# hyye/lio-mapping

Measured on AMD Instinct MI355X. Metric: sliding-window solves/sec, 64-line 130k-pt scans, window=15 (opt_window=5), higher is better.
Workload: dtype f64 (solve) / f32 (features); 1 GPU; HDL-64E outdoor_test_config_64, S_outdoor ray-cast scans, window_size=15 opt_window_size=5, one SolveOptimization per step, clouds resident in HBM; n_lidar_residuals=78236, local_map_points=76752, surf_stack_points=19386, parallelism=1 window

## Files before the change

### lio-mapping_amd/csrc/cloud_kernels.h

```cpp
#pragma once
#include <algorithm>
#include <cmath>
#include <cstdint>

#include "dev.h"
#include "hmath.h"

namespace lio {

struct VoxParams {
  float mn[3], mx[3];
  int minb[3], divb[3];
  int overflow;
  int n_valid;
};

struct Affine3f { float m[12]; };

#define LIO_MAX_FRAMES 32

struct ConcatSeg { const float4 *src; int n; int dst_off; int identity; int set_intensity; float intensity; Affine3f tf; };
struct ConcatArgs { ConcatSeg seg[LIO_MAX_FRAMES]; int nseg; int total; };
void launch_transform_concat(const ConcatArgs &a, float4 *dst, hipStream_t s);

void launch_deskew_to_end(float4 *pts, int n, const float q[4], const float p[3], float time_factor, hipStream_t s, bool keep_intensity = false);
void launch_rigid_map(const float4 *in, int n, const float q[4], const float p[3], float4 *out, hipStream_t s);

inline int cloud_bounds_blocks(int n) { return std::max(1, std::min(cdiv(n, 256), 512)); }
struct BoundsSeg { const float4 *pts; int n, nb, off; };
void launch_seg_bounds(const BoundsSeg *d_segs, int nseg, int max_nb, float *partial, float inv_leaf, VoxParams *d_out, hipStream_t s);

#define VSORT_CAP 4096
#define VSORT_MEAN 384
#define VSORT_OVERSAMPLE 8
#define VSORT_MAX_BUCKETS 1024
#define VSORT_MAX_N (VSORT_MAX_BUCKETS * VSORT_MEAN)
enum VoxSortPath { VSORT_PATH_SAMPLE = 0, VSORT_PATH_SINGLE = 1, VSORT_PATH_LIBRARY = 2 };
inline int vsort_buckets(size_t n) { return int((n + VSORT_MEAN - 1) / VSORT_MEAN); }

class VoxelGridDev {
 public:
  void sort_stats(unsigned long long out[3]) const { for (int k = 0; k < 3; ++k) out[k] = n_path_[k]; }
  int sort_pairs_hook(const uint32_t *keys, size_t n, uint32_t *keys_out, uint32_t *vals_out, hipStream_t s);
  size_t run(const float4 *in, size_t n, float leaf, DBuf<float4> &out, hipStream_t s, VoxParams *host_params = nullptr);
  void launch(const float4 *in, size_t n, float leaf, DBuf<float4> &out, hipStream_t s);
  size_t finish(VoxParams *host_params = nullptr);
  void set_host_signal(bool on) { use_signal_ = on; }
  VoxelGridDev() = default;
  VoxelGridDev(const VoxelGridDev &) = delete;
  VoxelGridDev &operator=(const VoxelGridDev &) = delete;

 private:
  const float4 *p_in_ = nullptr; size_t p_n_ = 0; DBuf<float4> *p_out_ = nullptr; hipStream_t p_stream_ = nullptr;
  float p_leaf_ = 0.f;
  void enqueue(bool exact, bool library);
  void reserve_sort(size_t n, hipStream_t s);
  int enqueue_sort(size_t n, hipStream_t s, bool library);
  DBuf<uint32_t> splitters_;
  DBuf<int> fill_;
  DBuf<unsigned long long> pairs_;
  int last_path_ = VSORT_PATH_LIBRARY;
  unsigned long long n_path_[3] = {0, 0, 0};
  HostBuf<char> h_mail_;
  int *h_count_ = nullptr;
  VoxParams *h_params_ = nullptr;
  DBuf<float> partial_;
  DBuf<VoxParams> params_;
  DBuf<uint32_t> keys_, keys2_, vals_, vals2_;
  DBuf<int> count_, tile_heads_;
  DBuf<char> tmp_;
  unsigned *h_flag_ = nullptr;
  unsigned seq_ = 0;
  HostSignal sig_{};
  bool use_signal_ = true;
};

struct GridDesc {
  int origin[3];
  int dims[3];
  float inv_cell;
  int n_points;
};

inline float knn_cell_edge(float min_match_sq_dis) { return std::sqrt(min_match_sq_dis) * 1.0001f + 1e-6f; }
inline float scan_to_map_cell_edge(float min_match_sq_dis) { return std::sqrt(min_match_sq_dis) * 1.0001f; }
inline void host_cloud_bounds(const float *xyzi, size_t n, float mn[3], float mx[3]) {
  for (int d = 0; d < 3; ++d) { mn[d] = 0.f; mx[d] = 0.f; }
  bool first = true;
  for (size_t i = 0; i < n; ++i) {
    const float *p = xyzi + 4 * i;
    if (!std::isfinite(p[0]) || !std::isfinite(p[1]) || !std::isfinite(p[2])) continue;
    for (int d = 0; d < 3; ++d) {
      if (first || p[d] < mn[d]) mn[d] = p[d];
      if (first || p[d] > mx[d]) mx[d] = p[d];
    }
    first = false;
  }
}
inline size_t grid_extent(GridDesc &g, const float mn[3], const float mx[3], float cell) {
  g.inv_cell = 1.0f / cell;
  size_t ncells = 1;
  for (int d = 0; d < 3; ++d) {
    const int lo = int(std::floor(mn[d] * g.inv_cell)) - 1, hi = int(std::floor(mx[d] * g.inv_cell)) + 1;
    g.origin[d] = lo; g.dims[d] = hi - lo + 1;
    ncells *= size_t(g.dims[d]);
  }
  return ncells;
}

class KnnGrid {
 public:
  void build(const float4 *pts, size_t n, const float mn[3], const float mx[3], float cell, hipStream_t s);
  const float4 *sorted() const { return sorted_.p; }
  const int *cells() const { return cells_.p; }
  const GridDesc &desc() const { return desc_; }

 private:
  GridDesc desc_{};
  DBuf<uint32_t> keys_, keys2_, vals_, vals2_;
  DBuf<float4> sorted_;
  DBuf<int> cells_, cnt_;
  bool cnt_dirty_ = false;
  DBuf<char> tmp_;
};

struct GridSeg { const float4 *pts; GridDesc g; int pt_off, cell_off, ncells; };
class GridBatch {
 public:
  void *begin(size_t head_bytes, int clouds);
  const void *head_dev() const { return d_tab_.p; }
  void add(const float4 *pts, int n);
  const VoxParams *bounds(hipStream_t s, float inv_leaf = 1.0f);
  void layout(float cell, size_t cells_cap);
  bool shared(int i) const { return gseg(i).pt_off >= 0; }
  const GridDesc &desc(int i) const { return gseg(i).g; }
  const float4 *sorted(int) const { return sorted_.p; }
  const int *cells(int i) const { return cells_.p + gseg(i).cell_off; }
// ... 149 lines not shown
```

### lio-mapping_amd/csrc/cloud_kernels.hip

```cpp
#include <cstring>
#include <hip/hip_runtime.h>
#include <rocprim/rocprim.hpp>

#include <cfloat>
#include <climits>

#include "cloud_kernels.h"
#include "cloud_device.h"

namespace lio {

__global__ void k_transform_concat(ConcatArgs a, float4 *__restrict__ dst) {
  int gid = blockIdx.x * blockDim.x + threadIdx.x;
  if (gid >= a.total) return;
  dst[gid] = concat_point(a.seg, a.nseg, gid, nullptr);
}

void launch_transform_concat(const ConcatArgs &a, float4 *dst, hipStream_t s) {
  if (a.total <= 0) return;
  hipLaunchKernelGGL(k_transform_concat, dim3(cdiv(a.total, 256)), dim3(256), 0, s, a, dst);
  LIO_HIP(hipGetLastError());
}

template <bool KEEP>
__global__ void __launch_bounds__(256) k_deskew_to_end(float4 *pts, int n, Quat<float> qe, Vec3<float> te, float time_factor) {
  int i = blockIdx.x * blockDim.x + threadIdx.x;
  if (i >= n) return;
  pts[i] = deskew_to_end_point<KEEP>(pts[i], qe, te, time_factor);
}
void launch_deskew_to_end(float4 *pts, int n, const float q[4], const float p[3], float time_factor, hipStream_t s, bool keep_intensity) {
  if (n <= 0) return;
  const Quat<float> qe(q[3], q[0], q[1], q[2]);
  const Vec3<float> te(p[0], p[1], p[2]);
  if (keep_intensity) hipLaunchKernelGGL(k_deskew_to_end<true>, dim3(cdiv(n, 256)), dim3(256), 0, s, pts, n, qe, te, time_factor);
  else hipLaunchKernelGGL(k_deskew_to_end<false>, dim3(cdiv(n, 256)), dim3(256), 0, s, pts, n, qe, te, time_factor);
  LIO_HIP(hipGetLastError());
}

__global__ void __launch_bounds__(256) k_rigid_map(const float4 *__restrict__ in, int n, Quat<float> q, Vec3<float> t, float4 *__restrict__ out) {
  const int i = blockIdx.x * blockDim.x + threadIdx.x;
  if (i >= n) return;
  out[i] = rigid_map_point(in[i], q, t);
}
void launch_rigid_map(const float4 *in, int n, const float q[4], const float p[3], float4 *out, hipStream_t s) {
  if (n <= 0) return;
  hipLaunchKernelGGL(k_rigid_map, dim3(cdiv(n, 256)), dim3(256), 0, s, in, n, Quat<float>(q[3], q[0], q[1], q[2]), Vec3<float>(p[0], p[1], p[2]), out);
  LIO_HIP(hipGetLastError());
}

__global__ void __launch_bounds__(VOX_TILE) k_seg_bounds(const BoundsSeg *__restrict__ recs, float *__restrict__ partial) {
  const BoundsSeg r = recs[blockIdx.y];
  if (int(blockIdx.x) >= r.nb) return;
  cloud_bounds_block(r.pts, r.n, blockIdx.x, r.nb, partial + (size_t(r.off) + blockIdx.x) * 8);
}
__global__ void __launch_bounds__(VOX_TILE) k_seg_bounds_fold(const BoundsSeg *__restrict__ recs, const float *__restrict__ partial, float inv_leaf,
                                                              VoxParams *__restrict__ out) {
  const BoundsSeg r = recs[blockIdx.x];
  VoxParams v;
  if (vox_fold_bounds(partial + size_t(r.off) * 8, r.nb, inv_leaf, v)) out[blockIdx.x] = v;
}
void launch_seg_bounds(const BoundsSeg *d_segs, int nseg, int max_nb, float *partial, float inv_leaf, VoxParams *d_out, hipStream_t s) {
  hipLaunchKernelGGL(k_seg_bounds, dim3(max_nb, nseg), dim3(VOX_TILE), 0, s, d_segs, partial);
  hipLaunchKernelGGL(k_seg_bounds_fold, dim3(nseg), dim3(VOX_TILE), 0, s, d_segs, partial, inv_leaf, d_out);
  LIO_HIP(hipGetLastError());
}
__global__ void __launch_bounds__(VOX_TILE) k_cloud_bounds(const float4 *__restrict__ pts, int n, float *__restrict__ partial) {
  cloud_bounds_block(pts, n, blockIdx.x, gridDim.x, partial + size_t(blockIdx.x) * 8);
}
__global__ void __launch_bounds__(VOX_TILE) k_cloud_bounds_fold(const float *__restrict__ partial, int nb, float inv_leaf, VoxParams *out) {
  VoxParams v;
  if (vox_fold_bounds(partial, nb, inv_leaf, v)) *out = v;
}

__global__ void k_vox_keys(const float4 *__restrict__ pts, int n, float inv_leaf, const VoxParams *__restrict__ vp,
                           uint32_t *__restrict__ keys, uint32_t *__restrict__ vals) {
  int i = blockIdx.x * blockDim.x + threadIdx.x;
  if (i >= n) return;
  float4 p = pts[i];
  uint32_t key = VOX_KEY_NONE;
  if (finite3(p)) {
    int i0 = int(floorf(p.x * inv_leaf) - float(vp->minb[0]));
    int i1 = int(floorf(p.y * inv_leaf) - float(vp->minb[1]));
    int i2 = int(floorf(p.z * inv_leaf) - float(vp->minb[2]));
    key = uint32_t(i0 + i1 * vp->divb[0] + i2 * vp->divb[0] * vp->divb[1]);
  }
  keys[i] = key;
  vals[i] = uint32_t(i);
}

__global__ void __launch_bounds__(VOX_TILE) k_vox_keys_abs(const float4 *__restrict__ pts, int n, float inv_leaf, uint32_t *__restrict__ keys,
                                                          uint32_t *__restrict__ vals, float *__restrict__ partial, int *__restrict__ range_overflow) {
  const int i = blockIdx.x * VOX_TILE + threadIdx.x;
  float mn[3] = {FLT_MAX, FLT_MAX, FLT_MAX}, mx[3] = {-FLT_MAX, -FLT_MAX, -FLT_MAX};
  float cnt = 0;
  if (i < n) {
    keys[i] = vox_take_point<10, VOX_KEY_NONE>(pts[i], inv_leaf, mn, mx, cnt, range_overflow);
    vals[i] = uint32_t(i);
  }
  vox_block_partial(mn, mx, cnt, partial + size_t(blockIdx.x) * 8);
}

__global__ void __launch_bounds__(VSORT_THREADS) k_vsort_splitters(const uint32_t *__restrict__ keys, int n, int NB, uint32_t *__restrict__ splitters,
                                                                  int *__restrict__ fill, int *__restrict__ overflow) {
  __shared__ __attribute__((aligned(16))) uint32_t ss[VSORT_OVERSAMPLE * VSORT_MAX_BUCKETS];
  if (blockIdx.x == 0) {
    for (int b = threadIdx.x; b < NB; b += VSORT_THREADS) fill[b] = 0;
    if (threadIdx.x == 0) *overflow = 0;
  }
  vsort_pick_splitters<VSORT_OVERSAMPLE>(keys, n, NB, ss, splitters);
}

__global__ void __launch_bounds__(VSORT_SCATTER_THREADS) k_vsort_scatter(const uint32_t *__restrict__ keys, int n, int NB,
                                                                        const uint32_t *__restrict__ splitters, int *__restrict__ fill,
                                                                        unsigned long long *__restrict__ pairs, int *__restrict__ overflow) {
  __shared__ uint32_t sspl[VSORT_MAX_BUCKETS];
  __shared__ int scnt[VSORT_MAX_BUCKETS], sbase[VSORT_MAX_BUCKETS];
  const int tid = threadIdx.x;
  for (int b = tid; b < NB; b += VSORT_SCATTER_THREADS) { scnt[b] = 0; if (b < NB - 1) sspl[b] = splitters[b]; }
  __syncthreads();
  uint32_t key[VSORT_SCATTER_ITEMS];
  int bucket[VSORT_SCATTER_ITEMS], rank[VSORT_SCATTER_ITEMS];
#pragma unroll
  for (int r = 0; r < VSORT_SCATTER_ITEMS; ++r) {
    const int i = (blockIdx.x * VSORT_SCATTER_ITEMS + r) * VSORT_SCATTER_THREADS + tid;
    bucket[r] = -1;
    if (i < n) {
      key[r] = keys[i];
      bucket[r] = vsort_bucket_of(sspl, NB, key[r]);
      rank[r] = atomicAdd(&scnt[bucket[r]], 1);
    }
  }
  __syncthreads();
  for (int b = tid; b < NB; b += VSORT_SCATTER_THREADS) {
    const int c = scnt[b];
    if (c > 0) sbase[b] = atomicAdd(&fill[b], c);
  }
  __syncthreads();
#pragma unroll
  for (int r = 0; r < VSORT_SCATTER_ITEMS; ++r) {
    if (bucket[r] < 0) continue;
    const int i = (blockIdx.x * VSORT_SCATTER_ITEMS + r) * VSORT_SCATTER_THREADS + tid;
    const int pos = sbase[bucket[r]] + rank[r];
    if (pos < VSORT_CAP) pairs[size_t(bucket[r]) * VSORT_CAP + pos] = (static_cast<unsigned long long>(key[r]) << 32) | uint32_t(i);
    else *overflow = 1;
  }
}

__global__ void __launch_bounds__(VSORT_THREADS) k_vsort_buckets(const unsigned long long *__restrict__ pairs, const int *__restrict__ fill, int NB, int n,
                                                                const int *__restrict__ overflow, uint32_t *__restrict__ keys_out,
                                                                uint32_t *__restrict__ vals_out) {
  __shared__ unsigned long long sp[VSORT_CAP];
  __shared__ int swave[VSORT_THREADS / 64];
  const int b = blockIdx.x, tid = threadIdx.x;
  if (*overflow) {
    const int chunk = (n + NB - 1) / NB;
    for (int i = b * chunk + tid; i < min(n, (b + 1) * chunk); i += VSORT_THREADS) keys_out[i] = VOX_KEY_NONE;
    return;
  }
  int before = 0;
  for (int j = tid; j < b; j += VSORT_THREADS) before += min(fill[j], VSORT_CAP);
#pragma unroll
  for (int o = 32; o > 0; o >>= 1) before += __shfl_xor(before, o, 64);
  if ((tid & 63) == 0) swave[tid >> 6] = before;
  const int m = min(fill[b], VSORT_CAP);
  __syncthreads();
  int off = 0;
#pragma unroll
  for (int w = 0; w < VSORT_THREADS / 64; ++w) off += swave[w];
  const unsigned long long *src = pairs + size_t(b) * VSORT_CAP;
  switch (vsort_items_for(m)) {
    case 1: vsort_pairs_sort_store<1>(src, m, sp, keys_out, vals_out, off); break;
    case 2: vsort_pairs_sort_store<2>(src, m, sp, keys_out, vals_out, off); break;
    case 4: vsort_pairs_sort_store<4>(src, m, sp, keys_out, vals_out, off); break;
    case 8: vsort_pairs_sort_store<8>(src, m, sp, keys_out, vals_out, off); break;
    default: vsort_pairs_sort_store<16>(src, m, sp, keys_out, vals_out, off); break;
  }
}

__global__ void __launch_bounds__(VSORT_THREADS) k_vsort_single(const uint32_t *__restrict__ keys, int n, int *__restrict__ overflow,
                                                               uint32_t *__restrict__ keys_out, uint32_t *__restrict__ vals_out) {
  __shared__ __attribute__((aligned(16))) uint32_t ss[VSORT_CAP];
  if (blockIdx.x == 0 && threadIdx.x == 0) *overflow = 0;
  const int S = (n + 3) & ~3;
  for (int t = threadIdx.x; t < S; t += VSORT_THREADS) ss[t] = t < n ? keys[t] : VOX_KEY_NONE;
  __syncthreads();
  const int i = blockIdx.x * (VSORT_THREADS / VSORT_RANK_LANES) + int(threadIdx.x) / VSORT_RANK_LANES, part = int(threadIdx.x) % VSORT_RANK_LANES;
  const unsigned long long mine = i < n ? (static_cast<unsigned long long>(ss[i]) << 32) | uint32_t(i) : 0ull;
  const int rank = vsort_rank_of(ss, S, part, mine);
  if (part == 0 && i < n) { keys_out[rank] = uint32_t(mine >> 32); vals_out[rank] = uint32_t(i); }
}

__global__ void __launch_bounds__(VOX_TILE) k_vox_tile_heads(const uint32_t *__restrict__ keys, int n, int *__restrict__ tile_heads,
                                                             const float *__restrict__ partial, int npartial, float inv_leaf, VoxParams *__restrict__ params) {
  if (blockIdx.x == gridDim.x - 1) {
    if (npartial <= 0) return;
    VoxParams v;
    if (vox_fold_bounds(partial, npartial, inv_leaf, v)) *params = v;
    return;
  }
  vox_tile_head_count(keys, n, blockIdx.x, tile_heads + blockIdx.x);
}

struct VoxMail { int count; VoxParams params; int range_overflow; int sort_overflow; };
__global__ void __launch_bounds__(VOX_TILE) k_vox_centroids(const float4 *__restrict__ pts, const uint32_t *__restrict__ keys,
                                                            const uint32_t *__restrict__ vals, const int *__restrict__ tile_heads, int n,
                                                            float4 *__restrict__ out, int *__restrict__ count, const VoxParams *__restrict__ params,
                                                            int *__restrict__ range_overflow, const int *__restrict__ sort_overflow, VoxMail *mail,
                                                            HostSignal sig) {
  const VoxSlot r = vox_centroid_tile(pts, keys, vals, tile_heads, n, blockIdx.x, out);
  if (blockIdx.x == gridDim.x - 1) {
    __shared__ VoxMail smail;
    const int tid = threadIdx.x;
    if (tid == VOX_TILE - 1) {
      const int total = r.pos + (r.head ? 1 : 0);
      *count = total;
      smail.count = total; smail.params = *params; smail.range_overflow = *range_overflow; smail.sort_overflow = *sort_overflow;
      if (sig.flag) *range_overflow = 0;
    }
    if (sig.flag) {
      __syncthreads();
      if (tid < 64) post_host_mail(sig, mail, &smail, int(sizeof(VoxMail) / 4), tid);
    }
  }
}

void VoxelGridDev::launch(const float4 *in, size_t n, float leaf, DBuf<float4> &out, hipStream_t s) {
  p_in_ = in; p_n_ = n; p_out_ = &out; p_stream_ = s; p_leaf_ = leaf;
  if (n == 0) return;
  enqueue(false, false);
}

void VoxelGridDev::enqueue(bool exact, bool library) {
  const float4 *in = p_in_;
  const size_t n = p_n_;
  DBuf<float4> &out = *p_out_;
  hipStream_t s = p_stream_;
  const int ni = int(n);
  const float inv_leaf = 1.0f / p_leaf_;
  const int nkb = cdiv(ni, VOX_TILE);
  partial_.reserve(size_t(std::max(nkb, 512)) * 8);
  params_.reserve(1);
  reserve_sort(n, s);
  out.reserve(n);
  if (!h_count_) {
    h_mail_.alloc(256, hipHostMallocCoherent, true);
    static_assert(sizeof(VoxMail) <= 128, "mailbox layout");
    h_count_ = reinterpret_cast<int *>(h_mail_.p);
    h_params_ = reinterpret_cast<VoxParams *>(h_count_ + 1);
    h_flag_ = reinterpret_cast<unsigned *>(reinterpret_cast<char *>(h_count_) + 128);
  }
  int *d_range = count_.p + 1;
  if (!use_signal_) LIO_HIP(hipMemsetAsync(d_range, 0, sizeof(int), s));
  int npartial = 0;
  if (exact) {
    const int nb = cloud_bounds_blocks(ni);
    hipLaunchKernelGGL(k_cloud_bounds, dim3(nb), dim3(VOX_TILE), 0, s, in, ni, partial_.p);
    hipLaunchKernelGGL(k_cloud_bounds_fold, dim3(1), dim3(VOX_TILE), 0, s, partial_.p, nb, inv_leaf, params_.p);
    hipLaunchKernelGGL(k_vox_keys, dim3(cdiv(ni, 256)), dim3(256), 0, s, in, ni, inv_leaf, params_.p, keys_.p, vals_.p);
  } else {
    hipLaunchKernelGGL(k_vox_keys_abs, dim3(nkb), dim3(VOX_TILE), 0, s, in, ni, inv_leaf, keys_.p, vals_.p, partial_.p, d_range);
    npartial = nkb;
  }
  last_path_ = enqueue_sort(n, s, library);
  const int ntiles = cdiv(ni, VOX_TILE);
  tile_heads_.reserve(ntiles);
  hipLaunchKernelGGL(k_vox_tile_heads, dim3(ntiles + 1), dim3(VOX_TILE), 0, s, keys2_.p, ni, tile_heads_.p, partial_.p, npartial, inv_leaf, params_.p);
  sig_ = HostSignal();
  if (use_signal_) { sig_.flag = h_flag_; sig_.seq = ++seq_; }

  hipLaunchKernelGGL(k_vox_centroids, dim3(ntiles), dim3(VOX_TILE), 0, s, in, keys2_.p, vals2_.p, tile_heads_.p, ni, out.p, count_.p, params_.p, d_range,
                     count_.p + 2, reinterpret_cast<VoxMail *>(h_count_), sig_);
  LIO_HIP(hipGetLastError());
  if (!sig_.flag) {
    VoxMail *m = reinterpret_cast<VoxMail *>(h_count_);
    LIO_HIP(hipMemcpyAsync(&m->count, count_.p, sizeof(int), hipMemcpyDeviceToHost, s));
    LIO_HIP(hipMemcpyAsync(&m->params, params_.p, sizeof(VoxParams), hipMemcpyDeviceToHost, s));
    LIO_HIP(hipMemcpyAsync(&m->range_overflow, d_range, sizeof(int), hipMemcpyDeviceToHost, s));
    LIO_HIP(hipMemcpyAsync(&m->sort_overflow, count_.p + 2, sizeof(int), hipMemcpyDeviceToHost, s));
  }
}

void VoxelGridDev::reserve_sort(size_t n, hipStream_t s) {
  keys_.reserve(n); keys2_.reserve(n); vals_.reserve(n); vals2_.reserve(n);
  if (count_.cap < 3) { count_.reserve(3); LIO_HIP(hipMemsetAsync(count_.p, 0, count_.cap * sizeof(int), s)); }
}

int VoxelGridDev::enqueue_sort(size_t n, hipStream_t s, bool library) {
  const int ni = int(n);
  int *d_overflow = count_.p + 2;
  if (library || n > size_t(VSORT_MAX_N)) {
    LIO_HIP(hipMemsetAsync(d_overflow, 0, sizeof(int), s));
    size_t tmp_bytes = 0;
    LIO_HIP(rocprim::radix_sort_pairs(nullptr, tmp_bytes, keys_.p, keys2_.p, vals_.p, vals2_.p, n, 0, 32, s));
    tmp_.reserve(tmp_bytes + 256);
    LIO_HIP(rocprim::radix_sort_pairs(tmp_.p, tmp_bytes, keys_.p, keys2_.p, vals_.p, vals2_.p, n, 0, 32, s));
    return VSORT_PATH_LIBRARY;
  }
  if (ni <= VSORT_CAP) {
    hipLaunchKernelGGL(k_vsort_single, dim3(cdiv(ni, VSORT_THREADS / VSORT_RANK_LANES)), dim3(VSORT_THREADS), 0, s, keys_.p, ni, d_overflow, keys2_.p, vals2_.p);
    return VSORT_PATH_SINGLE;
  }
  const int NB = vsort_buckets(n);
  splitters_.reserve(NB); fill_.reserve(NB); pairs_.reserve(size_t(NB) * VSORT_CAP);
  hipLaunchKernelGGL(k_vsort_splitters, dim3(cdiv(VSORT_OVERSAMPLE * NB, VSORT_THREADS / VSORT_RANK_LANES)), dim3(VSORT_THREADS), 0, s, keys_.p, ni, NB,
                     splitters_.p, fill_.p, d_overflow);
  hipLaunchKernelGGL(k_vsort_scatter, dim3(cdiv(ni, VSORT_SCATTER_THREADS * VSORT_SCATTER_ITEMS)), dim3(VSORT_SCATTER_THREADS), 0, s, keys_.p, ni, NB,
                     splitters_.p, fill_.p, pairs_.p, d_overflow);
  hipLaunchKernelGGL(k_vsort_buckets, dim3(NB), dim3(VSORT_THREADS), 0, s, pairs_.p, fill_.p, NB, ni, d_overflow, keys2_.p, vals2_.p);
  return VSORT_PATH_SAMPLE;
}

int VoxelGridDev::sort_pairs_hook(const uint32_t *keys, size_t n, uint32_t *keys_out, uint32_t *vals_out, hipStream_t s) {
  reserve_sort(n, s);
  std::vector<uint32_t> iota(n);
  for (size_t i = 0; i < n; ++i) iota[i] = uint32_t(i);
  LIO_HIP(hipMemcpyAsync(keys_.p, keys, n * sizeof(uint32_t), hipMemcpyHostToDevice, s));
  LIO_HIP(hipMemcpyAsync(vals_.p, iota.data(), n * sizeof(uint32_t), hipMemcpyHostToDevice, s));
  int path = enqueue_sort(n, s, false);
  LIO_HIP(hipGetLastError());
  int overflow = 0;
  LIO_HIP(hipMemcpyAsync(&overflow, count_.p + 2, sizeof(int), hipMemcpyDeviceToHost, s));
  LIO_HIP(hipStreamSynchronize(s));
  if (overflow) path = enqueue_sort(n, s, true);
  LIO_HIP(hipMemcpyAsync(keys_out, keys2_.p, n * sizeof(uint32_t), hipMemcpyDeviceToHost, s));
  LIO_HIP(hipMemcpyAsync(vals_out, vals2_.p, n * sizeof(uint32_t), hipMemcpyDeviceToHost, s));
  LIO_HIP(hipStreamSynchronize(s));
  return path;
}

size_t VoxelGridDev::finish(VoxParams *host_params) {
  if (p_n_ == 0) {
    if (host_params) std::memset(host_params, 0, sizeof(*host_params));
    return 0;
  }
  const VoxMail *m = reinterpret_cast<const VoxMail *>(h_count_);
  bool redone = false, exact = false, library = false;
  for (;;) {
    if (sig_.flag) wait_host_signal(sig_, p_stream_);
    else LIO_HIP(hipStreamSynchronize(p_stream_));
    if (m->range_overflow == 1 && !exact) {
      exact = true;
      enqueue(exact, library);
      redone = true;
// ... 565 lines not shown
```

### lio-mapping_amd/csrc/estimator.h

```cpp
#pragma once
#include <climits>
#include <condition_variable>
#include <exception>
#include <functional>
#include <memory>
#include <mutex>
#include <thread>
#include <vector>

#include "../../include/lio_c.h"
#include "cloud_kernels.h"
#include "cloud_src.h"
#include "host_init.h"
#include "host_solver.h"
#include "batch_kernels.h"
#include "resident_moments.h"
#include "solve_step.h"

namespace lio {

typedef Rigid<float> Rigidf;
typedef Rigid<double> Rigidd;

struct EstConfig {
// ... 172 lines not shown
  Rigidf CompactPredict(const Rigidf &transform_sum);
  bool PushFrame(const Rigidf &transform_in, CloudSrc surf, CloudSrc corner, double stamp);
  bool PushRefused() const { return inited_ && (cfg_.enable_deskew || cfg_.cutoff_deskew) && !cfg_.cutoff_deskew && imu_stamped_.empty(); }
  void PushFrameBegin(const Rigidf &transform_in, size_t n_surf, size_t n_corner, double stamp, PushPlan &pl);
  void PushFrameEnd(PushPlan &pl);
  bool SlideBegin(ConcatArgs &ca);
  void SlideEnd(bool concat, const ConcatArgs &ca);
  float4 *slide_dst() const { return scratch_cloud_.buf.p; }
  void SetMapRefresh(bool on, MappingDev *map);
  bool map_refresh() const { return map_refresh_; }
  int RefreshMap();
  const MapRefreshRecord &last_refresh() const { return last_refresh_; }
  const DeviceCloud *OptSurfCloud(long surf_frame) const;
  size_t CopyCloudToHost(const DeviceCloud *c, float *out);
  MappingDev *map_ = nullptr;
  void SetFullCloud(bool on, MappingDev *map);
  bool full_cloud() const { return full_cloud_; }
  void CorrectNewestFull();
  const FullEntry *FullEntryOf(int frame) const;
  Rigidf OptPose(int i) const;
  bool RegisteredFull(int frame, Rigidf *T, size_t *n, float *out);
  bool RunInitialization();
  void SetStatesFromLaser();
  bool SolveOptimization(lio_solve_report *rep) { return solve_hook_ ? solve_hook_(rep) : SolveOptimizationHost(rep); }
  bool SolveOptimizationHost(lio_solve_report *rep);
  std::function<bool(lio_solve_report *)> solve_hook_;
  void SlideWindow();
  void BuildLocalMap(lio_solve_report *rep);

  bool BatchEligible() const;
  int BatchDescribe(BatchWin &bw);
  bool BatchPackProblem(int bpf, DevProblem &pb, DevState &st, std::shared_ptr<MargPrior> *prior);
  int device_solve_limit_ = 6;
  bool BatchFinish(const DevState &st, const std::shared_ptr<MargPrior> &prior_used, lio_solve_report &R, DevMarg &mg, std::shared_ptr<MargPrior> *shell);
  void ApplyOdomState(const OdomState &st);
  int FillMomentFrames(MomentFrame *fr, int slot_base) const;

  void SetWindow(const double *Ps, const double *Rs, const double *Vs, const double *Bas, const double *Bgs, const double g[3]);
  void SetSurfStack(int frame, const float *xyzi, size_t n);
  size_t GetSurfStack(int frame, float *out);
  void SetPreintegration(int frame, std::shared_ptr<Preintegration> p) { pre_integrations_[frame] = std::move(p); frames_dirty_ = true; }
  void BeginFrame(const V3d &acc, const V3d &gyr);
  size_t GetLocalMap(float *out);
  size_t GetFeatures(int frame, double *pt, double *co, double *sc);
  int EvalLidarMoments(int n_passes, const double *Rt, double *out);
  void Snapshot();
  bool Restore();
  bool CopySnapshotOf(Estimator &src);
  bool BenchBatchedMoments(int n_windows, int reps, double *avg_ms, double *bytes);

  EstConfig cfg_;
  int W_, Wo_;
  std::vector<V3d> Ps_, Vs_, Bas_, Bgs_;
  std::vector<M3d> Rs_;
  V3d g_vec_, acc_last_, gyr_last_;
  Rigidf transform_lb_, laser_odom_transform_;
  bool inited_ = false, first_imu_ = false, init_local_map_ = false, convergence_flag_ = false;
  int cir_buf_count_ = 0;
  std::vector<LaserFrame> all_laser_transforms_;
  int n_state_ = 0;
  int n_frames_ = 0;
  int laser_odom_recv_count_ = 0, extrinsic_stage_ = 2;
  double initial_time_ = -1;
  M3d R_WI_;
  enum { EV_SKIPPED = 0, EV_FILLING = 1, EV_INIT_FAILED = 2, EV_INITIALISED = 3, EV_SOLVED = 4 };
  int last_event_ = EV_SKIPPED;
  std::shared_ptr<MargPrior> last_marg_;
  MargWorker marg_worker_;
  bool async_marg_ = true;
  unsigned marg_epoch_ = 0, marg_task_epoch_ = 0;
  void JoinMarg(bool materialize = true) {
    std::shared_ptr<MargPrior> r;
    const bool discard = marg_task_epoch_ != marg_epoch_;
    try {
      if (marg_worker_.join(r) && !discard) last_marg_ = std::move(r);
    } catch (...) {
      if (!discard) throw;
    }
    if (materialize && last_marg_) last_marg_->materialize();
  }
  std::vector<std::shared_ptr<Preintegration>> pre_integrations_;
  std::shared_ptr<Preintegration> tmp_pre_integration_;
  int laser_odom_iters_ = 0, laser_odom_kz_ = 0;
  double dbg_eval_ms_ = 0, dbg_sync_ms_ = 0; int dbg_eval_n_ = 0;
  KernelTimers timers_;
  int shard_rank_ = 0, shard_world_ = 1;
  lio_allreduce_fn allreduce_ = nullptr;
  void *allreduce_user_ = nullptr;
  void *rccl_comm_ = nullptr;
  bool Sharded() const { return shard_world_ > 1 && (allreduce_ || rccl_comm_); }
  ResidentMoments resident_;
  hipStream_t stream() const { return stream_; }

 private:
  friend class EstimatorBatch;
  struct ResidentScope { Estimator *e; ~ResidentScope() { e->resident_.End(e->stream_); } };
  void Init(), Close() noexcept;
  struct HostState;
  Rigidd LidarPose(int i, const Rigidd &lb) const;
  Rigidf RelTransform(int i, const Rigidd &T_pivot, const Rigidd &lb) const;
  bool KeepFeatures() const { return cfg_.keep_features && cfg_.imu_factor; }
  WindowPlan PlanWindow(int first_frame);
  void AssembleSystem(WindowParams &P, WindowSystem &sys) const;
  void VectorToParams(WindowParams &P) const;
  void ParamsToVector(const WindowParams &P);
  void FillMomentArgs(MomentArgs &ma, int &max_slots) const;
  void LidarEval(const WindowParams &P, std::vector<FrameMoments> &m);
  void LidarLaunch(const WindowParams &P);
  void LidarLaunchMoments(const MomentArgs &ma, bool reduce = true);
  void LidarWait(std::vector<FrameMoments> &m, bool reduce = true);
  bool LidarWaitFrame(int i, FrameMoments &fm);
  void PushCloud(DeviceCloud &&c, size_t n, int n_before);
  void PushState(int from);

  hipStream_t stream_ = nullptr, stream2_ = nullptr;
  bool owns_stream_ = true;
  void AdoptStream(hipStream_t s);
  void ReleaseAdoptedStream();
  void FusePivotOnce();
  hipEvent_t ev_fork_ = nullptr, ev_join_ = nullptr;
  std::vector<DeviceCloud> stacks_;
  std::vector<size_t> size_surf_stack_;
  std::vector<StampedPose> imu_stamped_;
  DeviceCloud local_, local_filtered_, scratch_cloud_, upload_;
  VoxelGridDev vox_;
  KnnGrid grid_;
  DBuf<uint8_t> f_valid_;
  DBuf<float4> f_coef_;
  DBuf<float> f_score_;
  std::vector<int> slot_off_, nslots_;
  size_t total_slots_ = 0;
  EstimatorBatch *feat_batch_ = nullptr;
  int feat_batch_w_ = -1;
  DBuf<float> d_transforms_;
  DBuf<OdomState> d_odom_;
  DBuf<double> d_odom_partials_, d_moment_partials_, d_moment_out_;
  HostBuf<double> h_moment_out_;
  HostBuf<OdomState> h_odom_;
  HostBuf<unsigned> h_signal_;
  unsigned signal_seq_[2] = {0, 0};
  bool host_signal_ = true;
  int device_id_ = 0;
  HostSignal moment_signal_{};
  bool frames_dirty_ = true;
  std::unique_ptr<HostState> snap_;
  std::vector<DeviceCloud> snap_stacks_;
  bool map_refresh_ = false;
  std::vector<OptSlot> opt_ring_;
  long frame_seq_ = 0;
  std::shared_ptr<DeviceCloud> corner_last_;
  std::vector<std::shared_ptr<DeviceCloud>> corner_pool_;
  std::shared_ptr<DeviceCloud> AcquireCornerCloud();
  DeviceCloud opt_evicted_, snap_opt_evicted_;
  long opt_evicted_frame_ = -1;
  DeviceCloud upload_corner_;
  VoxelGridDev vox_corner_;
  MapRefreshRecord last_refresh_;
  Rigidf OptPose0() const { return OptPose(W_ - Wo_); }
  bool full_cloud_ = false;
  std::vector<FullEntry> full_ring_;
  DBuf<float4> full_out_;
  void PushFull(const Rigidf &tes);
  void DropFullRing();
};

}
// ... 1 lines not shown
```

### lio-mapping_amd/csrc/estimator.hip

```cpp
#include "estimator.h"
#include "est_batch.h"
#include "mapping.h"
#include "marg_kernels.h"
#include "rccl_comm.h"

#include <atomic>
#include <cfloat>
#include <climits>
#include <cstring>

namespace lio {

static const bool g_debug_timing = std::getenv("LIO_DEBUG_TIMING") != nullptr;

static V3d R2ypr(const M3d &R) {
  V3d n(R(0, 0), R(1, 0), R(2, 0)), o(R(0, 1), R(1, 1), R(2, 1)), a(R(0, 2), R(1, 2), R(2, 2));
  double y = atan2(n.y, n.x);
  double p = atan2(-n.z, n.x * cos(y) + n.y * sin(y));
  double r = atan2(a.x * sin(y) - a.y * cos(y), -o.x * sin(y) + o.y * cos(y));
  return V3d(y, p, r) / M_PI * 180.0;
}
static M3d ypr2R(const V3d &ypr) {
  double y = ypr.x / 180.0 * M_PI, p = ypr.y / 180.0 * M_PI, r = ypr.z / 180.0 * M_PI;
  M3d Rz, Ry, Rx;
// ... 541 lines not shown
  const Rigidd lb = toDouble(transform_lb_);
  const Qd rot_li = fromRot(Rs_[i] * toRot(normalized(conj(lb.rot))));
  const V3d pos_li = Ps_[i] - rotate(rot_li, lb.pos);
  return toFloat(Rigidd(rot_li, pos_li));
}

int Estimator::RefreshMap() {
  if (!map_) throw std::runtime_error("RefreshMap: the estimator has no map");
  last_refresh_ = MapRefreshRecord();
  last_refresh_.have = true;
  if (opt_ring_.empty()) return 0;
  OptSlot &s0 = opt_ring_.front();
  s0.transform = OptPose0();
  last_refresh_.slot = s0;
  if (int(opt_ring_.size()) != Wo_ + 1 || s0.mask) return 0;
  const DeviceCloud *surf = OptSurfCloud(s0.surf_frame);
  if (!surf) throw std::runtime_error("RefreshMap: slot 0's surf stack has left the window");
  const DeviceCloud *cor = s0.corner.get();
  map_->UpdateMapDatabase(cor ? cor->buf.p : nullptr, cor ? cor->n : 0, surf->buf.p, surf->n, s0.valid_idx.data(), s0.valid_idx.size(), s0.transform,
                          s0.cen, stream_);
  last_refresh_.applied = 1;
  return 1;
}

void Estimator::FusePivotOnce() {
  if (init_local_map_) return;
  const int pivot = W_ - Wo_;
  const Rigidd lb = toDouble(transform_lb_);
  const Rigidd T_pivot = LidarPose(pivot, lb);
  ConcatArgs ca{};
  int total = 0;
  for (int i = 0; i <= pivot; ++i) {
    ConcatSeg &sg = ca.seg[ca.nseg++];
    sg.src = stacks_[i].buf.p; sg.n = int(stacks_[i].n); sg.dst_off = total; sg.set_intensity = 0; sg.intensity = 0; sg.identity = 0;
    sg.tf = affineOf(RelTransform(i, T_pivot, lb));
    total += sg.n;
  }
  ca.total = total;
  scratch_cloud_.buf.reserve(std::max(total, 1));
  launch_transform_concat(ca, scratch_cloud_.buf.p, stream_);
  scratch_cloud_.n = size_t(total);
  scratch_cloud_.id = ++g_content_id;
  std::swap(stacks_[pivot], scratch_cloud_);
  init_local_map_ = true;
}

WindowPlan Estimator::PlanWindow(int first_frame) {
  WindowPlan pl{};
  const int pivot = pl.pivot = W_ - Wo_;
  const Rigidd lb = toDouble(transform_lb_);
  const Rigidd T_pivot = LidarPose(pivot, lb);
  pl.keep_mult = KeepFeatures() ? 10 : 1;
  total_slots_ = 0;
  for (int i = 0; i <= W_; ++i) {
    slot_off_[i] = int(total_slots_);
    nslots_[i] = 0;
    if (i > pivot) { nslots_[i] = int(stacks_[i].n) * ((i == W_) ? pl.keep_mult : 1); total_slots_ += size_t(nslots_[i]); }
    pl.max_slots = std::max(pl.max_slots, nslots_[i]);
    if (i < first_frame) continue;
    const Rigidf tf = RelTransform(i, T_pivot, lb);
    const Rigidf T = fromAffine(linearOf(tf), tf.pos);
    float *o = pl.tf[i];
    o[0] = T.rot.x; o[1] = T.rot.y; o[2] = T.rot.z; o[3] = T.rot.w; o[4] = T.pos.x; o[5] = T.pos.y; o[6] = T.pos.z;
    if (i < pivot || i == W_) continue;
    ConcatSeg &sg = pl.seg[pl.nseg++];
    sg.src = stacks_[i].buf.p; sg.n = int(stacks_[i].n); sg.dst_off = pl.n_local;
    if (i == pivot) { sg.identity = 1; sg.set_intensity = 0; sg.intensity = 0; }
    else { sg.identity = 0; sg.set_intensity = 1; sg.intensity = float(i); sg.tf = affineOf(tf); }
    pl.n_local += sg.n;
  }
  return pl;
}

void Estimator::BuildLocalMap(lio_solve_report *rep) {
  const double t0 = now_ms();
  feat_batch_ = nullptr; feat_batch_w_ = -1;
  FusePivotOnce();
  const WindowPlan pl = PlanWindow(0);
  const int pivot = pl.pivot, total = pl.n_local, keep_mult = pl.keep_mult;
  ConcatArgs ca{};
  std::copy(pl.seg, pl.seg + pl.nseg, ca.seg);
  ca.nseg = pl.nseg; ca.total = total;
  local_.buf.reserve(std::max(total, 1));
  int th = timers_.begin(KT_CONCAT, 32.0 * total, stream_);
  launch_transform_concat(ca, local_.buf.p, stream_);
  timers_.end(th, stream_);
  local_.n = size_t(total);
  VoxParams vp;
  th = timers_.begin(KT_VOXEL, 32.0 * total, stream_);
  local_filtered_.n = vox_.run(local_.buf.p, local_.n, cfg_.surf_filter_size, local_filtered_.buf, stream_, &vp);
  timers_.end(th, stream_);
  const double t1 = now_ms();
  th = timers_.begin(KT_KNN_GRID, 32.0 * double(local_filtered_.n), stream_);
  grid_.build(local_filtered_.buf.p, local_filtered_.n, vp.mn, vp.mx, knn_cell_edge(cfg_.min_match_sq_dis), stream_);
  timers_.end(th, stream_);
  f_valid_.reserve(std::max<size_t>(total_slots_, 1)); f_coef_.reserve(std::max<size_t>(total_slots_, 1)); f_score_.reserve(std::max<size_t>(total_slots_, 1));
  SolveSetup su{};
  su.ntf = W_ + 1;
  std::memcpy(su.tf, pl.tf, sizeof(float) * 8 * size_t(W_ + 1));
  std::memcpy(su.odom_T, pl.tf[W_], 8 * sizeof(float));
  su.set_odom = cfg_.imu_factor ? 1 : 0;
  d_transforms_.reserve(size_t(W_ + 1) * 8);
  launch_solve_setup(su, d_transforms_.p, d_odom_.p, f_valid_.p, total_slots_, stream_);
  FeatArgs fa{};
  fa.min_match_sq_dis = cfg_.min_match_sq_dis; fa.min_plane_dis = cfg_.min_plane_dis;
  const int last_static = cfg_.imu_factor ? W_ - 1 : W_;
  for (int i = pivot + 1; i <= last_static; ++i) {
    FeatFrame &f = fa.fr[fa.nframes++];
    f.stack = stacks_[i].buf.p; f.M = int(stacks_[i].n); f.slot_off = slot_off_[i]; f.tf_index = i;
    fa.max_M = std::max(fa.max_M, f.M);
  }
  {
    double mq = 0;
    for (int k = 0; k < fa.nframes; ++k) mq += fa.fr[k].M;
    hipStream_t sf = cfg_.imu_factor ? stream2_ : stream_;
    if (sf != stream_) {
      LIO_HIP(hipEventRecord(ev_fork_, stream_));
      LIO_HIP(hipStreamWaitEvent(sf, ev_fork_, 0));
    }
    th = timers_.begin(KT_FEATURES, 16.0 * (mq + double(local_filtered_.n)) + 40.0 * mq + 32.0 * mq, sf);
    launch_features(fa, d_transforms_.p, grid_.sorted(), grid_.cells(), grid_.desc(), f_valid_.p, f_coef_.p, f_score_.p, nullptr, sf);
    timers_.end(th, sf);
    if (sf != stream_) LIO_HIP(hipEventRecord(ev_join_, sf));
  }
  laser_odom_iters_ = 0; laser_odom_kz_ = 0;
  if (cfg_.imu_factor) {
    OdomState st{};
    bool have_state = false;
    std::memcpy(st.T, pl.tf[W_], 8 * sizeof(float));
    const int M = int(stacks_[W_].n);
    const bool mail = host_signal_ && !timers_.on;
    HostSignal sig{};
    if (M > 0) {
      const int lpq = 8;
      const int nb = odom_round_blocks(M, lpq);
      d_odom_partials_.reserve(size_t(nb) * 28);
      FeatArgs fo{};
      fo.min_match_sq_dis = cfg_.min_match_sq_dis; fo.min_plane_dis = cfg_.min_plane_dis;
      fo.nframes = 1; fo.max_M = M;
      fo.fr[0].stack = stacks_[W_].buf.p; fo.fr[0].M = M; fo.fr[0].tf_index = 0; fo.fr[0].slot_off = slot_off_[W_];
      const int chunk_end[4] = {3, 5, 7, 10};
      int chunk = 0;
      for (int iter = 0; iter < 10; ++iter) {
        if (iter == chunk_end[chunk]) {
          if (mail) {
            wait_host_signal(sig, stream_);
          } else {
            LIO_HIP(hipMemcpyAsync(h_odom_.p, d_odom_.p, sizeof(st), hipMemcpyDeviceToHost, stream_));
            LIO_HIP(hipStreamSynchronize(stream_));
          }
          st = *h_odom_.p;
          if (st.converged) { have_state = true; break; }
          ++chunk;
        }
        if (mail) { sig.flag = h_signal_.p + 128; sig.seq = ++signal_seq_[1]; }
        const double ns = keep_mult > 1 ? double(iter + 1) * M : double(M);
        int t1h = timers_.begin(KT_ODOM_FEATURES, 16.0 * (double(M) + double(local_filtered_.n)) + 72.0 * M + 33.0 * ns, stream_);
        launch_odom_round(fo, slot_off_[W_], iter, keep_mult > 1 ? 1 : 0, d_odom_.p, grid_.sorted(), grid_.cells(), grid_.desc(), f_valid_.p, f_coef_.p,
                          f_score_.p, d_odom_partials_.p, stream_, mail ? h_odom_.p : nullptr, sig, lpq);
        timers_.end(t1h, stream_);
      }
    }
    LIO_HIP(hipStreamWaitEvent(stream_, ev_join_, 0));
    if (!have_state) {
      if (sig.flag) {
        wait_host_signal(sig, stream_);
      } else {
        LIO_HIP(hipMemcpyAsync(h_odom_.p, d_odom_.p, sizeof(st), hipMemcpyDeviceToHost, stream_));
        LIO_HIP(hipStreamSynchronize(stream_));
      }
      st = *h_odom_.p;
      timers_.resolve();
    }
    ApplyOdomState(st);
  } else {
    LIO_HIP(hipStreamSynchronize(stream_));
    timers_.resolve();
  }
  const double t2 = now_ms();
  if (rep) {
    rep->ms_build_map = t1 - t0; rep->ms_features = t2 - t1; rep->n_local_map = int(local_filtered_.n);
    rep->laser_odom_iterations = laser_odom_iters_; rep->laser_odom_kz = laser_odom_kz_;
  }
}

void Estimator::VectorToParams(WindowParams &P) const {
  const int pivot = W_ - Wo_;
  P.Wo = Wo_;
  P.pose.resize(Wo_ + 1); P.sb.resize(Wo_ + 1);
  for (int i = 0, oi = pivot; i <= Wo_; ++i, ++oi) {
    Qd q = fromRot(Rs_[oi]);
    P.pose[i] = {Ps_[oi].x, Ps_[oi].y, Ps_[oi].z, q.x, q.y, q.z, q.w};
    P.sb[i] = {Vs_[oi].x, Vs_[oi].y, Vs_[oi].z, Bas_[oi].x, Bas_[oi].y, Bas_[oi].z, Bgs_[oi].x, Bgs_[oi].y, Bgs_[oi].z};
  }
  P.ex = {transform_lb_.pos.x, transform_lb_.pos.y, transform_lb_.pos.z, transform_lb_.rot.x, transform_lb_.rot.y, transform_lb_.rot.z,
          transform_lb_.rot.w};
}

void Estimator::ParamsToVector(const WindowParams &P) {
  const int pivot = W_ - Wo_;
  const V3d origin_P0 = Ps_[pivot];
  const V3d origin_R0 = R2ypr(Rs_[pivot]);
  const M3d R00 = toRot(normalized(Qd(P.pose[0][6], P.pose[0][3], P.pose[0][4], P.pose[0][5])));
  const V3d origin_R00 = R2ypr(R00);
  const double y_diff = origin_R0.x - origin_R00.x;
  M3d rot_diff = ypr2R(V3d(y_diff, 0, 0));
  if (std::fabs(std::fabs(origin_R0.y) - 90) < 1.0 || std::fabs(std::fabs(origin_R00.y) - 90) < 1.0) rot_diff = Rs_[pivot] * transpose(R00);
  {
    Rigidd trans_pivot(fromRot(Rs_[pivot]), Ps_[pivot]);
    Rigidd trans_opt_pivot(fromRot(rot_diff * R00), origin_P0);
    for (int idx = 0; idx < pivot; ++idx) {
      Rigidd trans_idx(fromRot(Rs_[idx]), Ps_[idx]);
      Rigidd t = compose(compose(trans_opt_pivot, rinverse(trans_pivot)), trans_idx);
      Ps_[idx] = t.pos;
      Rs_[idx] = toRot(normalized(t.rot));
    }
  }
  for (int i = 0, oi = pivot; i <= Wo_; ++i, ++oi) {
    Qd qi(P.pose[i][6], P.pose[i][3], P.pose[i][4], P.pose[i][5]);
    Rs_[oi] = rot_diff * toRot(normalized(qi));
    Ps_[oi] = rot_diff * V3d(P.pose[i][0] - P.pose[0][0], P.pose[i][1] - P.pose[0][1], P.pose[i][2] - P.pose[0][2]) + origin_P0;
    Vs_[oi] = rot_diff * V3d(P.sb[i][0], P.sb[i][1], P.sb[i][2]);
    Bas_[oi] = V3d(P.sb[i][3], P.sb[i][4], P.sb[i][5]);
    Bgs_[oi] = V3d(P.sb[i][6], P.sb[i][7], P.sb[i][8]);
  }
  transform_lb_.pos = Vec3<float>(float(P.ex[0]), float(P.ex[1]), float(P.ex[2]));
  transform_lb_.rot = Quat<float>(float(P.ex[6]), float(P.ex[3]), float(P.ex[4]), float(P.ex[5]));
}

void Estimator::LidarEval(const WindowParams &P, std::vector<FrameMoments> &m) {
  LidarLaunch(P);
  LidarWait(m);
}

int Estimator::FillMomentFrames(MomentFrame *fr, int slot_base) const {
  int max_slots = 0;
  for (int i = 1; i <= Wo_; ++i) {
    MomentFrame &f = fr[i - 1];
    const int idx = W_ - Wo_ + i;
    f.stack = stacks_[idx].buf.p; f.M = std::max<int>(1, int(stacks_[idx].n)); f.slot_off = slot_base + slot_off_[idx]; f.nslots = nslots_[idx];
    f.slot_begin = 0; f.slot_end = f.nslots;
    if (Sharded()) {
      f.slot_begin = int((long long)f.nslots * shard_rank_ / shard_world_);
      f.slot_end = int((long long)f.nslots * (shard_rank_ + 1) / shard_world_);
    }
    max_slots = std::max(max_slots, f.nslots);
  }
  return max_slots;
}

void Estimator::FillMomentArgs(MomentArgs &ma, int &max_slots) const {
  ma = MomentArgs{};
  ma.nframes = Wo_;
  max_slots = FillMomentFrames(ma.fr, 0);
  ma.blocks_per_frame = moment_blocks_per_frame(max_slots);
  const int rb = resident_.Bpf(max_slots, ma.nframes);
  if (rb > 0) ma.blocks_per_frame = rb;
}

void Estimator::LidarLaunch(const WindowParams &P) {
  MomentArgs ma;
  int max_slots = 0;
  FillMomentArgs(ma, max_slots);
  for (int i = 1; i <= Wo_; ++i) relative_lidar_pose(P.pose[0].data(), P.pose[i].data(), P.ex.data(), ma.fr[i - 1].R, ma.fr[i - 1].t);
  LidarLaunchMoments(ma);
}
// ... 465 lines not shown
```

Before: 2450 solves/s.

## Fuse concat transform into voxel key intake and defer voxel finish

Merges the point transform/concat kernel with the voxel key computation, so each transformed point is written and keyed in one pass instead of being re-read. Voxel results are now finished after solve setup is queued, which hides part of the host wait behind more queued work. The odometry round loop moves into helper methods and now attaches a host signal only to the last launch of each chunk, reducing per-launch signalling. The helper split adds persistent state in the estimator and changes the stream ordering around the host mailbox.

```diff
diff --git a/lio-mapping_amd/csrc/cloud_kernels.h b/lio-mapping_amd/csrc/cloud_kernels.h
--- a/lio-mapping_amd/csrc/cloud_kernels.h
+++ b/lio-mapping_amd/csrc/cloud_kernels.h
@@ -45,6 +45,7 @@
   size_t run(const float4 *in, size_t n, float leaf, DBuf<float4> &out, hipStream_t s, VoxParams *host_params = nullptr);
   void launch(const float4 *in, size_t n, float leaf, DBuf<float4> &out, hipStream_t s);
   size_t finish(VoxParams *host_params = nullptr);
+  void launch_concat(const ConcatArgs &a, float4 *local, float leaf, DBuf<float4> &out, hipStream_t s);
   void set_host_signal(bool on) { use_signal_ = on; }
   VoxelGridDev() = default;
   VoxelGridDev(const VoxelGridDev &) = delete;
@@ -53,6 +54,7 @@
  private:
   const float4 *p_in_ = nullptr; size_t p_n_ = 0; DBuf<float4> *p_out_ = nullptr; hipStream_t p_stream_ = nullptr;
   float p_leaf_ = 0.f;
+  const ConcatArgs *p_concat_ = nullptr; float4 *p_local_ = nullptr;
   void enqueue(bool exact, bool library);
   void reserve_sort(size_t n, hipStream_t s);
   int enqueue_sort(size_t n, hipStream_t s, bool library);
diff --git a/lio-mapping_amd/csrc/cloud_kernels.hip b/lio-mapping_amd/csrc/cloud_kernels.hip
--- a/lio-mapping_amd/csrc/cloud_kernels.hip
+++ b/lio-mapping_amd/csrc/cloud_kernels.hip
@@ -95,6 +95,20 @@
   float cnt = 0;
   if (i < n) {
     keys[i] = vox_take_point<10, VOX_KEY_NONE>(pts[i], inv_leaf, mn, mx, cnt, range_overflow);
+    vals[i] = uint32_t(i);
+  }
+  vox_block_partial(mn, mx, cnt, partial + size_t(blockIdx.x) * 8);
+}
+
+__global__ void __launch_bounds__(VOX_TILE) k_intake_concat_keys(ConcatArgs a, float4 *__restrict__ dst, float inv_leaf, uint32_t *__restrict__ keys,
+                                                                uint32_t *__restrict__ vals, float *__restrict__ partial, int *__restrict__ range_overflow) {
+  const int i = blockIdx.x * VOX_TILE + threadIdx.x;
+  float mn[3] = {FLT_MAX, FLT_MAX, FLT_MAX}, mx[3] = {-FLT_MAX, -FLT_MAX, -FLT_MAX};
+  float cnt = 0;
+  if (i < a.total) {
+    const float4 o = concat_point(a.seg, a.nseg, i, nullptr);
+    dst[i] = o;
+    keys[i] = vox_take_point<10, VOX_KEY_NONE>(o, inv_leaf, mn, mx, cnt, range_overflow);
     vals[i] = uint32_t(i);
   }
   vox_block_partial(mn, mx, cnt, partial + size_t(blockIdx.x) * 8);
@@ -225,9 +239,17 @@
 }
 
 void VoxelGridDev::launch(const float4 *in, size_t n, float leaf, DBuf<float4> &out, hipStream_t s) {
-  p_in_ = in; p_n_ = n; p_out_ = &out; p_stream_ = s; p_leaf_ = leaf;
+  p_in_ = in; p_n_ = n; p_out_ = &out; p_stream_ = s; p_leaf_ = leaf; p_concat_ = nullptr;
   if (n == 0) return;
   enqueue(false, false);
+}
+
+void VoxelGridDev::launch_concat(const ConcatArgs &a, float4 *local, float leaf, DBuf<float4> &out, hipStream_t s) {
+  p_in_ = local; p_n_ = size_t(std::max(a.total, 0)); p_out_ = &out; p_stream_ = s; p_leaf_ = leaf;
+  if (p_n_ == 0) return;
+  p_concat_ = &a; p_local_ = local;
+  enqueue(false, false);
+  p_concat_ = nullptr;
 }
 
 void VoxelGridDev::enqueue(bool exact, bool library) {
@@ -258,7 +280,11 @@
     hipLaunchKernelGGL(k_cloud_bounds_fold, dim3(1), dim3(VOX_TILE), 0, s, partial_.p, nb, inv_leaf, params_.p);
     hipLaunchKernelGGL(k_vox_keys, dim3(cdiv(ni, 256)), dim3(256), 0, s, in, ni, inv_leaf, params_.p, keys_.p, vals_.p);
   } else {
-    hipLaunchKernelGGL(k_vox_keys_abs, dim3(nkb), dim3(VOX_TILE), 0, s, in, ni, inv_leaf, keys_.p, vals_.p, partial_.p, d_range);
+    if (p_concat_)
+      hipLaunchKernelGGL(k_intake_concat_keys, dim3(nkb), dim3(VOX_TILE), 0, s, *p_concat_, p_local_, inv_leaf, keys_.p, vals_.p, partial_.p,
+                         d_range);
+    else
+      hipLaunchKernelGGL(k_vox_keys_abs, dim3(nkb), dim3(VOX_TILE), 0, s, in, ni, inv_leaf, keys_.p, vals_.p, partial_.p, d_range);
     npartial = nkb;
   }
   last_path_ = enqueue_sort(n, s, library);
diff --git a/lio-mapping_amd/csrc/estimator.h b/lio-mapping_amd/csrc/estimator.h
--- a/lio-mapping_amd/csrc/estimator.h
+++ b/lio-mapping_amd/csrc/estimator.h
@@ -278,6 +278,17 @@
   std::vector<std::shared_ptr<Preintegration>> pre_integrations_;
   std::shared_ptr<Preintegration> tmp_pre_integration_;
   int laser_odom_iters_ = 0, laser_odom_kz_ = 0;
+  struct OdomRounds {
+    FeatArgs fo{};
+    int M = 0, keep = 0;
+    int lpq = 8;
+    int iter = 0, chunk = 0;
+    bool mail = false;
+    HostSignal sig{};
+  } odom_rounds_;
+  void QueueOdomChunk();
+  OdomState ReadOdomState();
+  void FinishOdomRounds();
   double dbg_eval_ms_ = 0, dbg_sync_ms_ = 0; int dbg_eval_n_ = 0;
   KernelTimers timers_;
   int shard_rank_ = 0, shard_world_ = 1;
diff --git a/lio-mapping_amd/csrc/estimator.hip b/lio-mapping_amd/csrc/estimator.hip
--- a/lio-mapping_amd/csrc/estimator.hip
+++ b/lio-mapping_amd/csrc/estimator.hip
@@ -647,26 +647,24 @@
   std::copy(pl.seg, pl.seg + pl.nseg, ca.seg);
   ca.nseg = pl.nseg; ca.total = total;
   local_.buf.reserve(std::max(total, 1));
-  int th = timers_.begin(KT_CONCAT, 32.0 * total, stream_);
-  launch_transform_concat(ca, local_.buf.p, stream_);
+  f_valid_.reserve(std::max<size_t>(total_slots_, 1)); f_coef_.reserve(std::max<size_t>(total_slots_, 1)); f_score_.reserve(std::max<size_t>(total_slots_, 1));
+  d_transforms_.reserve(size_t(W_ + 1) * 8);
+  VoxParams vp;
+  int th = timers_.begin(KT_VOXEL, 64.0 * total, stream_);
+  vox_.launch_concat(ca, local_.buf.p, cfg_.surf_filter_size, local_filtered_.buf, stream_);
   timers_.end(th, stream_);
   local_.n = size_t(total);
-  VoxParams vp;
-  th = timers_.begin(KT_VOXEL, 32.0 * total, stream_);
-  local_filtered_.n = vox_.run(local_.buf.p, local_.n, cfg_.surf_filter_size, local_filtered_.buf, stream_, &vp);
-  timers_.end(th, stream_);
-  const double t1 = now_ms();
-  th = timers_.begin(KT_KNN_GRID, 32.0 * double(local_filtered_.n), stream_);
-  grid_.build(local_filtered_.buf.p, local_filtered_.n, vp.mn, vp.mx, knn_cell_edge(cfg_.min_match_sq_dis), stream_);
-  timers_.end(th, stream_);
-  f_valid_.reserve(std::max<size_t>(total_slots_, 1)); f_coef_.reserve(std::max<size_t>(total_slots_, 1)); f_score_.reserve(std::max<size_t>(total_slots_, 1));
   SolveSetup su{};
   su.ntf = W_ + 1;
   std::memcpy(su.tf, pl.tf, sizeof(float) * 8 * size_t(W_ + 1));
   std::memcpy(su.odom_T, pl.tf[W_], 8 * sizeof(float));
   su.set_odom = cfg_.imu_factor ? 1 : 0;
-  d_transforms_.reserve(size_t(W_ + 1) * 8);
   launch_solve_setup(su, d_transforms_.p, d_odom_.p, f_valid_.p, total_slots_, stream_);
+  local_filtered_.n = vox_.finish(&vp);
+  const double t1 = now_ms();
+  th = timers_.begin(KT_KNN_GRID, 32.0 * double(local_filtered_.n), stream_);
+  grid_.build(local_filtered_.buf.p, local_filtered_.n, vp.mn, vp.mx, knn_cell_edge(cfg_.min_match_sq_dis), stream_);
+  timers_.end(th, stream_);
   FeatArgs fa{};
   fa.min_match_sq_dis = cfg_.min_match_sq_dis; fa.min_plane_dis = cfg_.min_plane_dis;
   const int last_static = cfg_.imu_factor ? W_ - 1 : W_;
@@ -690,54 +688,19 @@
   }
   laser_odom_iters_ = 0; laser_odom_kz_ = 0;
   if (cfg_.imu_factor) {
-    OdomState st{};
-    bool have_state = false;
-    std::memcpy(st.T, pl.tf[W_], 8 * sizeof(float));
-    const int M = int(stacks_[W_].n);
-    const bool mail = host_signal_ && !timers_.on;
-    HostSignal sig{};
-    if (M > 0) {
-      const int lpq = 8;
-      const int nb = odom_round_blocks(M, lpq);
-      d_odom_partials_.reserve(size_t(nb) * 28);
-      FeatArgs fo{};
-      fo.min_match_sq_dis = cfg_.min_match_sq_dis; fo.min_plane_dis = cfg_.min_plane_dis;
-      fo.nframes = 1; fo.max_M = M;
-      fo.fr[0].stack = stacks_[W_].buf.p; fo.fr[0].M = M; fo.fr[0].tf_index = 0; fo.fr[0].slot_off = slot_off_[W_];
-      const int chunk_end[4] = {3, 5, 7, 10};
-      int chunk = 0;
-      for (int iter = 0; iter < 10; ++iter) {
-        if (iter == chunk_end[chunk]) {
-          if (mail) {
-            wait_host_signal(sig, stream_);
-          } else {
-            LIO_HIP(hipMemcpyAsync(h_odom_.p, d_odom_.p, sizeof(st), hipMemcpyDeviceToHost, stream_));
-            LIO_HIP(hipStreamSynchronize(stream_));
-          }
-          st = *h_odom_.p;
-          if (st.converged) { have_state = true; break; }
-          ++chunk;
-        }
-        if (mail) { sig.flag = h_signal_.p + 128; sig.seq = ++signal_seq_[1]; }
-        const double ns = keep_mult > 1 ? double(iter + 1) * M : double(M);
-        int t1h = timers_.begin(KT_ODOM_FEATURES, 16.0 * (double(M) + double(local_filtered_.n)) + 72.0 * M + 33.0 * ns, stream_);
-        launch_odom_round(fo, slot_off_[W_], iter, keep_mult > 1 ? 1 : 0, d_odom_.p, grid_.sorted(), grid_.cells(), grid_.desc(), f_valid_.p, f_coef_.p,
-                          f_score_.p, d_odom_partials_.p, stream_, mail ? h_odom_.p : nullptr, sig, lpq);
-        timers_.end(t1h, stream_);
-      }
-    }
-    LIO_HIP(hipStreamWaitEvent(stream_, ev_join_, 0));
-    if (!have_state) {
-      if (sig.flag) {
-        wait_host_signal(sig, stream_);
-      } else {
-        LIO_HIP(hipMemcpyAsync(h_odom_.p, d_odom_.p, sizeof(st), hipMemcpyDeviceToHost, stream_));
-        LIO_HIP(hipStreamSynchronize(stream_));
-      }
-      st = *h_odom_.p;
-      timers_.resolve();
-    }
-    ApplyOdomState(st);
+    OdomRounds &r = odom_rounds_;
+    r = OdomRounds();
+    r.M = int(stacks_[W_].n);
+    r.keep = keep_mult > 1 ? 1 : 0;
+    r.mail = host_signal_ && !timers_.on;
+    if (r.M > 0) {
+      d_odom_partials_.reserve(size_t(odom_round_blocks(r.M, r.lpq)) * 28);
+      r.fo.min_match_sq_dis = cfg_.min_match_sq_dis; r.fo.min_plane_dis = cfg_.min_plane_dis;
+      r.fo.nframes = 1; r.fo.max_M = r.M;
+      r.fo.fr[0].stack = stacks_[W_].buf.p; r.fo.fr[0].M = r.M; r.fo.fr[0].tf_index = 0; r.fo.fr[0].slot_off = slot_off_[W_];
+      QueueOdomChunk();
+    }
+    FinishOdomRounds();
   } else {
     LIO_HIP(hipStreamSynchronize(stream_));
     timers_.resolve();
@@ -747,6 +710,50 @@
     rep->ms_build_map = t1 - t0; rep->ms_features = t2 - t1; rep->n_local_map = int(local_filtered_.n);
     rep->laser_odom_iterations = laser_odom_iters_; rep->laser_odom_kz = laser_odom_kz_;
   }
+}
+
+static const int kOdomChunkEnd[4] = {3, 5, 7, 10};
+void Estimator::QueueOdomChunk() {
+  OdomRounds &r = odom_rounds_;
+  for (; r.iter < kOdomChunkEnd[r.chunk]; ++r.iter) {
+    const bool posts = r.mail && r.iter + 1 == kOdomChunkEnd[r.chunk];
+    if (posts) { r.sig.flag = h_signal_.p + 128; r.sig.seq = ++signal_seq_[1]; }
+    const double ns = r.keep ? double(r.iter + 1) * r.M : double(r.M);
+    int t1h = timers_.begin(KT_ODOM_FEATURES, 16.0 * (double(r.M) + double(local_filtered_.n)) + 72.0 * r.M + 33.0 * ns, stream_);
+    launch_odom_round(r.fo, slot_off_[W_], r.iter, r.keep, d_odom_.p, grid_.sorted(), grid_.cells(), grid_.desc(), f_valid_.p, f_coef_.p, f_score_.p,
+                      d_odom_partials_.p, stream_, posts ? h_odom_.p : nullptr, posts ? r.sig : HostSignal(), r.lpq);
+    timers_.end(t1h, stream_);
+  }
+}
+
+OdomState Estimator::ReadOdomState() {
+  if (odom_rounds_.sig.flag) {
+    wait_host_signal(odom_rounds_.sig, stream_);
+  } else {
+    LIO_HIP(hipMemcpyAsync(h_odom_.p, d_odom_.p, sizeof(OdomState), hipMemcpyDeviceToHost, stream_));
+    LIO_HIP(hipStreamSynchronize(stream_));
+  }
+  return *h_odom_.p;
+}
+
+void Estimator::FinishOdomRounds() {
+  OdomRounds &r = odom_rounds_;
+  OdomState st{};
+  bool have_state = false;
+  if (r.M > 0) {
+    while (r.iter < 10) {
+      st = ReadOdomState();
+      if (st.converged) { have_state = true; break; }
+      ++r.chunk;
+      QueueOdomChunk();
+    }
+  }
+  LIO_HIP(hipStreamWaitEvent(stream_, ev_join_, 0));
+  if (!have_state) {
+    st = ReadOdomState();
+    timers_.resolve();
+  }
+  ApplyOdomState(st);
 }
 
 void Estimator::VectorToParams(WindowParams &P) const {
```

After: 2464 solves/s (median of 2 runs). No clear change (+0.6%).
